# HanzhiC/TexPose

Measured on AMD Instinct MI355X. Metric: rendered rays/sec (480x640x128 samples) + train iters/sec, higher is better.
Workload: dtype f32 carried as 2xf16 (f16x3 products, f32 accumulate); 1 GPU; Duck-like synthetic scene 480x640, 128 samples/ray, batch=1 image per GPU, forward render (render_by_slices mode='val', all pixels), per-sample outputs materialised; samples_per_ray=128, mlp_precision=f16x3, parallelism=images sharded across 1 GPU(s), no collective

## Files before the change

### texpose_amd/csrc/gen_wide_asm.py

```python
#!/usr/bin/env python3
import sys

NCH = 115

VB = 160
def F_hi(slot): return VB + 8 * slot
def F_lo(slot): return VB + 8 * slot + 4
XB = [VB + 32, VB + 48]
T = VB + 64
VR = VB + 68
HACC = VB + 72
CLOBBER_V = list(range(XB[0], VR + 3))
BA, BB = 92, 94
CLOBBER_S = [BA, BA + 1, BB, BB + 1]
SET = {"P": 0, "Q": 128}


def vr(lo, n=4):
    return "v[%d:%d]" % (lo, lo + n - 1)


def ar(set_base, tile):
    lo = set_base + 16 * tile
    return "a[%d:%d]" % (lo, lo + 15)
# ... 100 lines not shown


def dma_base():
    return ["s_lshl_b32 %[t0], %[dch], 15",
            "s_add_u32 s%d, %%[stream_lo], %%[t0]" % BA,
            "s_addc_u32 s%d, %%[stream_hi], 0" % (BA + 1),
            "s_add_u32 s%d, s%d, 0x1000" % (BB, BA),
            "s_addc_u32 s%d, s%d, 0" % (BB + 1, BA + 1)]


def dma_piece(e, k, dma_slot):
    if k == 0:
        e("s_mov_b32 m0, %%[m%da]" % dma_slot)
        e("s_nop 0")
    elif k == 4:
        e("s_add_i32 m0, %%[m%da], 0x1000" % dma_slot)
        e("s_nop 0")
    base = "s[%d:%d]" % ((BA, BA + 1) if k < 4 else (BB, BB + 1))
    e("global_load_lds_dwordx4 %%[laneoff], %s offset:%d" % (base, (k & 3) * 1024))


def ring_epilogue(e, n_chunks):
    e("s_waitcnt lgkmcnt(0)")
    e("s_add_i32 %%[chunk], %%[chunk], %d" % n_chunks)
    e("s_cmp_ge_i32 %[chunk], %[nch]")
    e("s_cselect_b32 %[t0], %[nch], 0")
    e("s_sub_i32 %[chunk], %[chunk], %[t0]")
    e("s_add_i32 %%[buf], %%[buf], %d" % (n_chunks % 3))
    e("s_cmp_ge_i32 %[buf], 3")
    e("s_cselect_b32 %[t0], 3, 0")
    e("s_sub_i32 %[buf], %[buf], %[t0]")


def refill(e, slot, pair, npairs, cur, nxt):
    addr, off = (VR + cur, pair * 2048) if pair < npairs else (VR + nxt, (pair - npairs) * 2048)
    e("ds_read_b128 %s, v%d offset:%d" % (vr(F_hi(slot)), addr, off))
    e("ds_read_b128 %s, v%d offset:%d" % (vr(F_lo(slot)), addr, off + 1024))


def publish(e, young):
    e("s_waitcnt vmcnt(%d) lgkmcnt(0)" % young)
    e("s_barrier")


def chunk_groups(e, npairs, ts, mf, fill, free_after, pieces_per_group, tail=None, head=None, young_extra=0):
    ngroups = npairs // 2
    cur, nxt, dma = ts % 3, (ts + 1) % 3, (ts + 2) % 3
    pub_group = (npairs - 4) // 2
    for g in range(ngroups):
        q = 2 * g
        sa, sb = q % 4, (q + 1) % 4
        lines = mf(g)
        gaps = fill(g)
        e("s_waitcnt lgkmcnt(4)")
        for i in range(6):
            e(lines[i])
            if i == 0:
                for k in range(pieces_per_group):
                    dma_piece(e, g * pieces_per_group + k, dma)
                if head is not None:
                    for ins in head(g):
                        e(ins)
            if i < 5:
                for ins in gaps[i]:
                    e(ins)
            if i + 1 == free_after[0]:
                if g == pub_group:
                    publish(e, (g + 1) * pieces_per_group + young_extra)
                refill(e, sa, q + 4, npairs, cur, nxt)
            if i + 1 == free_after[1]:
                refill(e, sb, q + 5, npairs, cur, nxt)
        if tail is not None:
            for ins in tail(g):
                e(ins)


def advance_dch():
    return ["s_add_i32 %[dch], %[dch], 1", "s_cmp_eq_u32 %[dch], %[nch]", "s_cselect_b32 %[dch], 0, %[dch]"]


def gen_wide(src, dst, rec=None):
    L = []
    e = L.append
    ring_prologue(e)
    cvf = (lambda *a: conv_rec(*a, mask=(rec == "mask"))) if rec else conv
    if rec:
        e("s_mov_b64 s[%d:%d], %%[rbase]" % (RB, RB + 1))
    for g in range(8):
        for ins in cvf(src, 0, g, 0):
            e(ins)
    if rec:
        for ins in rec_reads(src, 0):
            e(ins)
    for ins in dma_base():
        e(ins)
    for ts in range(8):
        bank = ts & 1

        def mf(g, bank=bank):
            s, t = g >> 2, (2 * g) & 7
            sa, sb = (2 * g) % 4, (2 * g + 1) % 4
            xh, xl = vr(XB[bank] + s * 4), vr(XB[bank] + 8 + s * 4)
            d0, d1 = ar(dst, t), ar(dst, t + 1)
            return [mfma(d0, vr(F_hi(sa)), xh), mfma(d1, vr(F_hi(sb)), xh), mfma(d0, vr(F_hi(sa)), xl),
                    mfma(d1, vr(F_hi(sb)), xl), mfma(d0, vr(F_lo(sa)), xh), mfma(d1, vr(F_lo(sb)), xh)]

        def fill(g, ts=ts, bank=bank):
            if rec:
                first, mid1, mid2, mid3, last = [], [], [], [], []
                if 1 <= g <= 4:
                    first = [rec_store(src, ts, g - 1)]
                if g == 5:
                    first = rec_advance()
                if g == 7 and ts < 7:
                    rd = rec_reads(src, ts + 1)
                    mid2, mid3 = mid2 + rd[0:2], mid3 + rd[2:4]
                    if rec == "mask" and not (ts & 1):
                        last = last + rec_mask_store(ts >> 1)
                if ts == 7:
                    return [first, mid1, mid2, mid3, last]
                cv = conv_rec(src, ts + 1, g, bank ^ 1, mask=(rec == "mask"))
                if rec == "mask":
                    return [first + cv[0:4], mid1 + cv[4:9], cv[9:14] + mid2, cv[14:18] + mid3, cv[18:19] + last]
                return [first + cv[0:4], mid1 + cv[4:8], cv[8:12] + mid2, cv[12:15] + mid3, last]
            if ts == 7:
                return [[], [], [], [], []]
            cv = conv(src, ts + 1, g, bank ^ 1)
            return [[], cv[0:4], cv[4:8], cv[8:12], cv[12:13]]

        def tail(g, ts=ts):
            out = []
            if ts < 7:
                if 1 <= g <= 3:
                    out.append(advance_dch()[g - 1])
                if g == 7:
                    out += dma_base()
            return out

        def head(g, ts=ts):
            if g != (6 if rec else 0):
                return []
            return ["ds_read_b128 a[%d:%d], %%[nbias] offset:%d" % (src + 16 * ts + 4 * k, src + 16 * ts + 4 * k + 3, ts * 64 + k * 16)
                    for k in range(4)]

        extra = 0
        if rec:
            extra = 4 + (1 if (ts & 1) and rec == "mask" else 0)
        chunk_groups(e, 16, ts, mf, fill, (5, 6), 1, tail, head, young_extra=extra)
    ring_epilogue(e, 8)
    return L


def gen_extra(dst, ks):
    L = []
    e = L.append
    ring_prologue(e)
    for s in range(ks):
        e("ds_read_b128 %s, %%[stage] offset:%d" % (vr(XB[0] + s * 4), s * 8192))
        e("ds_read_b128 %s, %%[stage] offset:%d" % (vr(XB[0] + 8 + s * 4), s * 8192 + 4096))
    for ins in dma_base():
        e(ins)
    e("s_waitcnt lgkmcnt(0)")

    def mf(g):
        s, t = g >> 2, (2 * g) & 7
        sa, sb = (2 * g) % 4, (2 * g + 1) % 4
        xh, xl = vr(XB[0] + s * 4), vr(XB[0] + 8 + s * 4)
        d0, d1 = ar(dst, t), ar(dst, t + 1)
        return [mfma(d0, vr(F_hi(sa)), xh), mfma(d1, vr(F_hi(sb)), xh), mfma(d0, vr(F_hi(sa)), xl),
                mfma(d1, vr(F_hi(sb)), xl), mfma(d0, vr(F_lo(sa)), xh), mfma(d1, vr(F_lo(sb)), xh)]

    chunk_groups(e, 8 * ks, 0, mf, lambda g: [[], [], [], [], []], (5, 6), 2 // ks)
    ring_epilogue(e, 1)
    return L


def gen_head(src, rec=False):
    L = []
    e = L.append
    ring_prologue(e)
    if rec:
# ... 366 lines not shown

        tail = advance_dch() + dma_base() if c < 3 else []
        chunk16(e, lg, c, 4, dst, lambda s, b=b: vr(XB[b] + 4 * s), fill, tail)
    ring_epilogue(e, 4)
    return L


def gen_extra16(dst, ks):
    L = []
    e = L.append
    lg = Lgkm()
    ring_prologue(e)
    for s in range(ks):
        e("ds_read_b128 %s, %%[stage] offset:%d" % (vr(XB[0] + 4 * s), s * 8192))
    for ins in dma_base():
        e(ins)
    e("s_waitcnt lgkmcnt(0)")
    chunk16(e, lg, 0, ks, dst, lambda s: vr(XB[0] + 4 * s), lambda q: [])
    ring_epilogue(e, 1)
    return L


def emit_macro(out, name, comment, lines):
    out.append("// " + comment)
    out.append("#define %s \\" % name)
    out.append(" \\\n".join('    "%s\\n"' % l for l in lines))
    out.append("")


def main():
    out = ["// GENERATED by gen_wide_asm.py -- do not edit.  See that file for the schedule.", "#pragma once",
           "#define TP_ASM_CLOBBERS " + ", ".join(['"v%d"' % v for v in CLOBBER_V] + ['"s%d"' % r for r in CLOBBER_S] + ['"a%d"' % a for a in range(256)]),
           "#define TP_ASM_ALL_AGPRS " + ", ".join('"a%d"' % a for a in range(256)),
           '#define TP_ASM_REC_CLOBBERS "v%d", "s%d", "s%d", "vcc"' % (MK, RB, RB + 1)]
    for s, d in (("Q", "P"), ("P", "Q")):
        emit_macro(out, "TP_ASM_WIDE_%s%s" % (s, d), "256 -> 256 layer: set %s -> set %s" % (s, d), gen_wide(SET[s], SET[d]))
        emit_macro(out, "TP_ASM_WIDE_%s%s_REC" % (s, d), "256 -> 256 layer: set %s -> set %s, recording set %s (values + ReLU sign words)" % (s, d, s),
                   gen_wide(SET[s], SET[d], rec="mask"))
    emit_macro(out, "TP_ASM_WIDE_QP_RECNM", "256 -> 256 layer: set Q -> set P, recording set Q (values only: the trunk feature)",
               gen_wide(SET["Q"], SET["P"], rec="nomask"))
    for d in ("P", "Q"):
        for ks in (1, 2):
            emit_macro(out, "TP_ASM_EXTRA%d_%s" % (ks, d), "%d extra k-step(s) into set %s" % (ks, d), gen_extra(SET[d], ks))
        emit_macro(out, "TP_ASM_HEAD_%s" % d, "narrow head over relu(set %s)" % d, gen_head(SET[d]))
        emit_macro(out, "TP_ASM_HEAD_%s_REC" % d, "narrow head over relu(set %s), recording set %s" % (d, d), gen_head(SET[d], rec=True))
        emit_macro(out, "TP_ASM_INIT_%s" % d, "seed set %s with the bias block" % d, gen_init(SET[d]))
        for t in range(8):
            emit_macro(out, "TP_ASM_READ_%s%d" % (d, t), "tile %d of set %s -> v[232:247]" % (t, d), gen_read_tile(SET[d], t))
    emit_macro(out, "TP_ASM_HEADV_P1", "fp32 VALU head, 1 row, over relu(set P)", gen_head_valu(SET["P"], HEADTAB_SIGMA))
    emit_macro(out, "TP_ASM_HEADV_P5", "fp32 VALU head, 5 rows, over relu(set P)", gen_head_valu(SET["P"], HEADTAB_TRANS))
    emit_macro(out, "TP_ASM_HEADV_Q3", "fp32 VALU head, 3 rows, over relu(set Q)", gen_head_valu(SET["Q"], HEADTAB_RGB))
    out.append("#define TP_HEADTAB_OFFSETS {%s}" % ", ".join(str(v) for v in HEADTAB_SIGMA + HEADTAB_TRANS + HEADTAB_RGB))
    emit_macro(out, "TP_ASM_STASH_Q", "set Q -> v[32:159]", gen_stash(SET["Q"]))
    emit_macro(out, "TP_ASM_RESTORE_P", "v[32:159] -> set P", gen_restore(SET["P"]))
    for s, d in (("Q", "P"), ("P", "Q")):
        emit_macro(out, "TP_ASM_WIDE16_%s%s" % (s, d), "f16: 256 -> 256 layer: set %s -> set %s" % (s, d), gen_wide16(SET[s], SET[d]))
    for d in ("P", "Q"):
        for ks in (1, 4):
            emit_macro(out, "TP_ASM_EXTRA16_%d_%s" % (ks, d), "f16: %d extra k-step(s) into set %s" % (ks, d), gen_extra16(SET[d], ks))
    emit_macro(out, "TP_ASM_DG_NARROW_P", "data gradient: set P = W3^T d (one k-step)", gen_dg_narrow(SET["P"]))
    emit_macro(out, "TP_ASM_DG_WIDE_PQ", "data gradient: set Q = W^T gated(set P), recording gated(set P)", gen_dg_wide(SET["P"], SET["Q"]))
    emit_macro(out, "TP_ASM_DG_WIDE_QP", "data gradient: set P = W^T gated(set Q), recording gated(set Q)", gen_dg_wide(SET["Q"], SET["P"]))
    emit_macro(out, "TP_ASM_DG_FINISH_P", "data gradient: record gated(set P)", gen_dg_finish(SET["P"]))
    sys.stdout.write("\n".join(out) + "\n")


if __name__ == "__main__":
    main()
```

### texpose_amd/csrc/mlp_fwd_f16x3.hip

```cpp
#include "mlp_mma.h"
#include "wide_asm.inc.h"
#include <type_traits>

namespace {
using namespace tp_layout;
using namespace tp_mma;

using half8 = __attribute__((ext_vector_type(8))) _Float16;
using half2v = __attribute__((ext_vector_type(2))) __fp16;

constexpr int kBiasPad = (kBiasFloats + 63) / 64 * 64;
constexpr int kStageHalves = 5 * 2 * kThreads * 8;

constexpr int kBufs = 3;
constexpr int kSaveFloats = 8 * kThreads;
constexpr int kLdsBytes = kBufs * kChunkFloats * 4 + kBiasPad * 4 + kStageHalves * 2 + kSaveFloats * 4;
constexpr float kInvScale = 1.0f / (float)(1 << kF16WeightShift);

using u32x4 = __attribute__((ext_vector_type(4))) unsigned int;
__device__ __forceinline__ half8 pack8(const half2v (&p)[4]) {
  const u32x4 w = {__builtin_bit_cast(unsigned int, p[0]), __builtin_bit_cast(unsigned int, p[1]),
                   __builtin_bit_cast(unsigned int, p[2]), __builtin_bit_cast(unsigned int, p[3])};
  return __builtin_bit_cast(half8, w);
}
// ... 28 lines not shown
  for (int q = 0; q < kDepth; ++q) frag_fetch(f, q, l + q * kPairHalves);
}

struct Guard { half2v m = {(__fp16)0.0f, (__fp16)0.0f}; };

__device__ __forceinline__ float softplus(float x) { return x > 20.0f ? x : log1pf(expf(x)); }
__device__ __forceinline__ float sigmoid(float x) { return 1.0f / (1.0f + expf(-x)); }


struct AsmCtx { unsigned lane16, laneoff, ldswave, stream_lo, stream_hi, bias0, stage0; int nch; };
__device__ __forceinline__ AsmCtx asm_ctx_now(const float* packed, int nch = kNumChunks) {
  extern __shared__ __attribute__((aligned(16))) float lds_base[];
  int tid = threadIdx.x;
  asm volatile("" : "+v"(tid));
  const unsigned lane = (unsigned)tid & 63u, hh = ((unsigned)tid >> 5) & 1u;
  const unsigned wave = (unsigned)__builtin_amdgcn_readfirstlane(tid >> 6);
  AsmCtx c;
  const unsigned lds0 = (unsigned)(uintptr_t)AS3(lds_base);
  c.lane16 = lds0 + lane * 16u;
  c.laneoff = lane * 16u;
  c.ldswave = lds0 + wave * 8192u;
  const uint64_t sw = (uint64_t)(uintptr_t)(packed + wave * 2048);
  c.stream_lo = (unsigned)sw;
  c.stream_hi = (unsigned)(sw >> 32);
  const unsigned bias_lds = lds0 + (unsigned)(kBufs * kChunkFloats) * 4u;
  c.bias0 = bias_lds + hh * 512u;
  c.stage0 = bias_lds + (unsigned)kBiasPad * 4u + (unsigned)tid * 16u;
  c.nch = nch;
  return c;
}
#define TP_RING(f)                                                                                                     \
  "+{v[160:163]}"(f.h[0]), "+{v[164:167]}"(f.l[0]), "+{v[168:171]}"(f.h[1]), "+{v[172:175]}"(f.l[1]),                  \
      "+{v[176:179]}"(f.h[2]), "+{v[180:183]}"(f.l[2]), "+{v[184:187]}"(f.h[3]), "+{v[188:191]}"(f.l[3])
#define TP_RING_STATE                                                                                                  \
  [chunk] "+s"(chunk), [buf] "+s"(buf), [r0] "=&s"(r0), [r1] "=&s"(r1), [r2] "=&s"(r2), [m0a] "=&s"(m0a),              \
      [m1a] "=&s"(m1a), [m2a] "=&s"(m2a), [dch] "=&s"(dch), [t0] "=&s"(t0)
#define TP_RING_INPUTS(c)                                                                                              \
  [lane16] "v"(c.lane16), [laneoff] "v"(c.laneoff), [ldswave] "s"(__builtin_amdgcn_readfirstlane(c.ldswave)),         \
      [stream_lo] "s"(__builtin_amdgcn_readfirstlane(c.stream_lo)),                                                    \
      [stream_hi] "s"(__builtin_amdgcn_readfirstlane(c.stream_hi)), [nch] "s"(c.nch)
#define TP_ASM_HACC "v232", "v233", "v234", "v235", "v236", "v237", "v238", "v239", "v240", "v241", "v242", "v243", "v244", "v245", "v246", "v247"
#define TP_RING_LOCALS                                                                                                 \
  int chunk = __builtin_amdgcn_readfirstlane(p.chunk), buf = __builtin_amdgcn_readfirstlane(p.buf);                    \
  int r0, r1, r2, m0a, m1a, m2a, dch, t0
#define TP_RING_DONE                                                                                                   \
  p.chunk = chunk;                                                                                                     \
  p.buf = buf

#define TP_SF_OUT(F)                                                                                                   \
  "={v[32:47]}"(F[0]), "={v[48:63]}"(F[1]), "={v[64:79]}"(F[2]), "={v[80:95]}"(F[3]), "={v[96:111]}"(F[4]),            \
      "={v[112:127]}"(F[5]), "={v[128:143]}"(F[6]), "={v[144:159]}"(F[7])
#define TP_SF_IN(F)                                                                                                    \
  "{v[32:47]}"(F[0]), "{v[48:63]}"(F[1]), "{v[64:79]}"(F[2]), "{v[80:95]}"(F[3]), "{v[96:111]}"(F[4]),                 \
      "{v[112:127]}"(F[5]), "{v[128:143]}"(F[6]), "{v[144:159]}"(F[7])
__device__ __forceinline__ void asm_stash_q(f32x16 (&F)[8]) { asm volatile(TP_ASM_STASH_Q : TP_SF_OUT(F) : : TP_ASM_ALL_AGPRS); }
__device__ __forceinline__ void asm_restore_p(const f32x16 (&F)[8]) { asm volatile(TP_ASM_RESTORE_P : : TP_SF_IN(F) : TP_ASM_ALL_AGPRS); }
template <bool SRC_Q>
__device__ __forceinline__ void asm_wide(Pipe& p, Frag& f, Guard& amax, const AsmCtx& c, int next_li) {
  TP_RING_LOCALS;
  const float kinv = kInvScale;
  const unsigned mask = 0xFFFFE000u;
  const unsigned nbias = c.bias0 + (unsigned)next_li * 1024u;
  if constexpr (SRC_Q)
    asm volatile(TP_ASM_WIDE_QP : TP_RING(f), TP_RING_STATE, [amax] "+v"(amax.m)
                 : TP_RING_INPUTS(c), [kinv] "s"(kinv), [mask] "s"(mask), [nbias] "v"(nbias)
                 : TP_ASM_CLOBBERS, TP_ASM_HACC, "memory", "scc");
  else
    asm volatile(TP_ASM_WIDE_PQ : TP_RING(f), TP_RING_STATE, [amax] "+v"(amax.m)
                 : TP_RING_INPUTS(c), [kinv] "s"(kinv), [mask] "s"(mask), [nbias] "v"(nbias)
                 : TP_ASM_CLOBBERS, TP_ASM_HACC, "memory", "scc");
  TP_RING_DONE;
}

template <bool SRC_Q>
__device__ __forceinline__ void asm_wide16(Pipe& p, Frag& f, Guard& amax, const AsmCtx& c, int next_li) {
  TP_RING_LOCALS;
  const unsigned nbias = c.bias0 + (unsigned)next_li * 1024u;
  if constexpr (SRC_Q)
    asm volatile(TP_ASM_WIDE16_QP : TP_RING(f), TP_RING_STATE, [amax] "+v"(amax.m)
                 : TP_RING_INPUTS(c), [nbias] "v"(nbias) : TP_ASM_CLOBBERS, "memory", "scc");
  else
    asm volatile(TP_ASM_WIDE16_PQ : TP_RING(f), TP_RING_STATE, [amax] "+v"(amax.m)
                 : TP_RING_INPUTS(c), [nbias] "v"(nbias) : TP_ASM_CLOBBERS, "memory", "scc");
  TP_RING_DONE;
}

struct RecCtx { unsigned recw, recr, ro0, ro1, mkoff; const float* rbase; };
__device__ __forceinline__ RecCtx rec_ctx_now(float* saved, int64_t tile, int slot) {
  extern __shared__ __attribute__((aligned(16))) float lds_base[];
  int tid = threadIdx.x;
  asm volatile("" : "+v"(tid));
  const unsigned lane = (unsigned)tid & 63u, j = (unsigned)tid & 31u, hh = ((unsigned)tid >> 5) & 1u;
  const unsigned wave = (unsigned)__builtin_amdgcn_readfirstlane(tid >> 6);
  const unsigned stg = (unsigned)(uintptr_t)AS3(lds_base) + (unsigned)(kBufs * kChunkFloats + kBiasPad) * 4u + wave * 1024u;
  RecCtx c;
  c.recw = stg + ((4u * hh) * 32u + j) * 4u;
  c.recr = stg + lane * 16u;
  c.ro0 = (unsigned)blk_off(0 + (int)(lane >> 3), (int)(lane & 7u) * 4) * 4u;
  c.ro1 = (unsigned)blk_off(8 + (int)(lane >> 3), (int)(lane & 7u) * 4) * 4u;
  static_assert(blk_off(16 + 3, 12) == blk_off(3, 12) + 512 && blk_off(24 + 6, 20) == blk_off(8 + 6, 20) + 512,
                "units 2 / 3 of a record tile sit 16 rows behind units 0 / 1 with the same swizzle");
  c.mkoff = (unsigned)((kMaskOff + ((slot > 0 ? slot : 1) - 1) * 256 - slot * kBlockFloats) * 4) + lane * 4u;
  const float* base = saved + (tile * 4 + (int64_t)wave) * (int64_t)kSavedGroupFloats + (int64_t)slot * kBlockFloats;
  const uint64_t b = (uint64_t)(uintptr_t)base;
  c.rbase = reinterpret_cast<const float*>((uint64_t)(unsigned)__builtin_amdgcn_readfirstlane((int)(unsigned)b) |
                                           ((uint64_t)(unsigned)__builtin_amdgcn_readfirstlane((int)(unsigned)(b >> 32)) << 32));
  return c;
}
#define TP_REC_INPUTS(r)                                                                                               \
  [recw] "v"(r.recw), [recr] "v"(r.recr), [ro0] "v"(r.ro0), [ro1] "v"(r.ro1), [mkoff] "v"(r.mkoff), [rbase] "s"(r.rbase)

template <class L>
constexpr int rec_kind_of() {
  if constexpr (std::is_same_v<L, int>) return 0;
  else return L::value == T0 ? 2 : (L::value == T1 || L::value == T2 || L::value == R1 || L::value == R2) ? 1 : 0;
}

template <bool SRC_Q, bool MASK>
__device__ __forceinline__ void asm_wide_rec(Pipe& p, Frag& f, Guard& amax, const AsmCtx& c, int next_li, const RecCtx& r) {
  TP_RING_LOCALS;
  const float kinv = kInvScale;
  const unsigned mask = 0xFFFFE000u;
  const unsigned nbias = c.bias0 + (unsigned)next_li * 1024u;
  static_assert(SRC_Q || MASK, "the mask-free variant exists for set Q only");
#define TP_WIDE_REC(TXT)                                                                                               \
  asm volatile(TXT : TP_RING(f), TP_RING_STATE, [amax] "+v"(amax.m)                                                    \
               : TP_RING_INPUTS(c), [kinv] "s"(kinv), [mask] "s"(mask), [nbias] "v"(nbias), TP_REC_INPUTS(r)           \
               : TP_ASM_CLOBBERS, TP_ASM_REC_CLOBBERS, "memory", "scc")
  if constexpr (SRC_Q && MASK) TP_WIDE_REC(TP_ASM_WIDE_QP_REC);
  else if constexpr (SRC_Q) TP_WIDE_REC(TP_ASM_WIDE_QP_RECNM);
  else TP_WIDE_REC(TP_ASM_WIDE_PQ_REC);
#undef TP_WIDE_REC
  TP_RING_DONE;
}

template <int KS, bool DST_P>
__device__ __forceinline__ void asm_extra(Pipe& p, Frag& f, const AsmCtx& c, int ks0) {
  TP_RING_LOCALS;
  const unsigned stage = c.stage0 + (unsigned)ks0 * 8192u;
#define TP_EXTRA(TXT)                                                                                                  \
  asm volatile(TXT : TP_RING(f), TP_RING_STATE : TP_RING_INPUTS(c), [stage] "v"(stage)                  \
               : TP_ASM_CLOBBERS, "memory", "scc")
  if constexpr (KS == 1 && DST_P) TP_EXTRA(TP_ASM_EXTRA1_P);
  else if constexpr (KS == 2 && DST_P) TP_EXTRA(TP_ASM_EXTRA2_P);
  else if constexpr (KS == 1) TP_EXTRA(TP_ASM_EXTRA1_Q);
  else TP_EXTRA(TP_ASM_EXTRA2_Q);
#undef TP_EXTRA
  TP_RING_DONE;
}

template <int KS, bool DST_P>
__device__ __forceinline__ void asm_extra16(Pipe& p, Frag& f, const AsmCtx& c, int ks0) {
  TP_RING_LOCALS;
  const unsigned stage = c.stage0 + (unsigned)ks0 * 8192u;
#define TP_EXTRA16(TXT)                                                                                                \
  asm volatile(TXT : TP_RING(f), TP_RING_STATE : TP_RING_INPUTS(c), [stage] "v"(stage) : TP_ASM_CLOBBERS, "memory", "scc")
  if constexpr (KS == 1 && DST_P) TP_EXTRA16(TP_ASM_EXTRA16_1_P);
  else if constexpr (KS == 4 && DST_P) TP_EXTRA16(TP_ASM_EXTRA16_4_P);
  else if constexpr (KS == 1) TP_EXTRA16(TP_ASM_EXTRA16_1_Q);
  else TP_EXTRA16(TP_ASM_EXTRA16_4_Q);
#undef TP_EXTRA16
  TP_RING_DONE;
}

template <bool SRC_P>
__device__ __forceinline__ f32x16 asm_head(Pipe& p, Frag& f, Guard& amax, const AsmCtx& c, float kinv = kInvScale) {
  TP_RING_LOCALS;
  const unsigned mask = 0xFFFFE000u;
  f32x16 acc;
  if constexpr (SRC_P)
    asm volatile(TP_ASM_HEAD_P : TP_RING(f), TP_RING_STATE, [amax] "+v"(amax.m), "=&{v[232:247]}"(acc)
                 : TP_RING_INPUTS(c), [kinv] "s"(kinv), [mask] "s"(mask) : TP_ASM_CLOBBERS, "memory", "scc");
  else
    asm volatile(TP_ASM_HEAD_Q : TP_RING(f), TP_RING_STATE, [amax] "+v"(amax.m), "=&{v[232:247]}"(acc)
                 : TP_RING_INPUTS(c), [kinv] "s"(kinv), [mask] "s"(mask) : TP_ASM_CLOBBERS, "memory", "scc");
  TP_RING_DONE;
  return acc;
}

struct Head4 { float a0, a1, a2, a3; };
template <bool SRC_P>
__device__ __forceinline__ Head4 asm_head_rec(Pipe& p, Frag& f, Guard& amax, const AsmCtx& c, const RecCtx& r) {
  TP_RING_LOCALS;
  const float kinv = kInvScale;
  const unsigned mask = 0xFFFFE000u;
  Head4 h;
#define TP_HEAD_REC(TXT)                                                                                               \
  asm volatile(TXT : TP_RING(f), TP_RING_STATE, [amax] "+v"(amax.m), "=&{v232}"(h.a0), "=&{v233}"(h.a1),               \
                     "=&{v234}"(h.a2), "=&{v235}"(h.a3)                                                                \
               : TP_RING_INPUTS(c), [kinv] "s"(kinv), [mask] "s"(mask), TP_REC_INPUTS(r)                               \
               : TP_ASM_CLOBBERS, TP_ASM_REC_CLOBBERS, "v236", "v237", "v238", "v239", "v240", "v241", "v242", "v243", \
                 "v244", "v245", "v246", "v247", "memory", "scc")
  if constexpr (SRC_P) TP_HEAD_REC(TP_ASM_HEAD_P_REC);
  else TP_HEAD_REC(TP_ASM_HEAD_Q_REC);
#undef TP_HEAD_REC
  TP_RING_DONE;
  return h;
}

struct Head5 { float r0, r1, r2, r3, r4; };
template <int WHICH>
__device__ __forceinline__ Head5 asm_head_valu(const Pipe& p, Frag& f, const AsmCtx& c) {
  int tid = threadIdx.x;
  asm volatile("" : "+v"(tid));
  const unsigned hw = c.stage0 - (unsigned)tid * 16u + (((unsigned)tid >> 5) & 1u) * 16u;
  const int buf = __builtin_amdgcn_readfirstlane(p.buf);
  int t0;
  Head5 h;
#define TP_HEADV(TXT)                                                                                                  \
  asm volatile(TXT : TP_RING(f), [t0] "=&s"(t0), "=&{v232}"(h.r0), "=&{v233}"(h.r1), "=&{v234}"(h.r2), "=&{v235}"(h.r3), \
                     "=&{v236}"(h.r4)                                                                                  \
               : [hw] "v"(hw), [lane16] "v"(c.lane16), [buf] "s"(buf)                                                  \
               : TP_ASM_CLOBBERS, "v231", "v237", "v238", "v239", "v240", "v241", "v242", "v243", "v244", "v245", "v246", "v247", \
                 "memory", "scc")
  if constexpr (WHICH == 0) TP_HEADV(TP_ASM_HEADV_P1);
  else if constexpr (WHICH == 1) TP_HEADV(TP_ASM_HEADV_P5);
  else TP_HEADV(TP_ASM_HEADV_Q3);
#undef TP_HEADV
  return h;
}

template <bool DST_P>
__device__ __forceinline__ void asm_init(const AsmCtx& c, int li) {
  const unsigned bias = c.bias0 + (unsigned)li * 1024u;
  if constexpr (DST_P) asm volatile(TP_ASM_INIT_P :: [bias] "v"(bias) : TP_ASM_CLOBBERS, "memory");
  else asm volatile(TP_ASM_INIT_Q :: [bias] "v"(bias) : TP_ASM_CLOBBERS, "memory");
}

struct Params {
  const float* packed;
  const float* center; const float* ray; const float* depth;
  const float* points; const float* ray_unit;
  const float* lat_trans; const float* lat_light;
  int B, R, N;
  int64_t n_samples, n_tiles;
  float* rgb; float* density; float* uncert; float* saved; float* workspace; int* status;
  const float* density_noise;
  unsigned int* act_max;
  const float* ray_bias;
};

__device__ __forceinline__ void stage(_Float16* st, int tid, int ks, int j, float v) {
  const _Float16 hi = (_Float16)v;
  st[((ks * 2 + 0) * kThreads + tid) * 8 + j] = hi;
  st[((ks * 2 + 1) * kThreads + tid) * 8 + j] = (_Float16)(v - (float)hi);
}

__device__ __forceinline__ void stage_slot(_Float16* st, int tid_lo, int slot, float v) {
  const int ks = slot >> 4, owner = tid_lo | ((slot & 8) << 2), jj = slot & 7;
  const _Float16 hi = (_Float16)v;
  st[((ks * 2 + 0) * kThreads + owner) * 8 + jj] = hi;
  st[((ks * 2 + 1) * kThreads + owner) * 8 + jj] = (_Float16)(v - (float)hi);
}

#define TP_THREAD_IDS                                                                                                  \
  int tid = threadIdx.x;                                                                                               \
  asm volatile("" : "+v"(tid));                                                                                        \
  const int lane = tid & 63, j = tid & 31, hh = (tid >> 5) & 1;                                                        \
  const int wave = __builtin_amdgcn_readfirstlane(tid >> 6);                                                           \
// ... 2 lines not shown

template <bool SAVE, bool RB = false, bool F16 = false>
__global__ __launch_bounds__(kThreads, 1) void mlp_fwd_f16x3_kernel(Params P) {
  static_assert(!(SAVE && RB), "the ray-bias stream has no recording variant");
  static_assert(!(SAVE && F16), "the single-product arithmetic is inference only");
  constexpr int NCH = F16 ? (RB ? kNumChunks16RB : kNumChunks16) : (RB ? kNumChunksRB : kNumChunks);
  constexpr int BIAS_NCH = RB ? kNumChunksRB : kNumChunks;
  constexpr float kSetScale = F16 ? 1.0f : (float)(1 << kF16WeightShift);
#define TP_CTX asm_ctx_now(P.packed, NCH)
  extern __shared__ __attribute__((aligned(16))) float lds[];
  const int tid = threadIdx.x, lane = tid & 63, wave = tid >> 6;
  float* bias_lds = lds + kBufs * kChunkFloats;
  _Float16* st = reinterpret_cast<_Float16*>(bias_lds + kBiasPad);

  Pipe p;
  p.stream = P.packed; p.lds = lds; p.chunk = 0; p.buf = 0; p.wave = __builtin_amdgcn_readfirstlane(wave); p.lane = lane;
  for (int i = tid; i < kBiasFloats; i += kThreads)
    bias_lds[i] = P.packed[(size_t)BIAS_NCH * kChunkFloats + i] * (i < kHeadBiasOff ? kSetScale : 1.0f);
  if constexpr (RB) {
    constexpr int kHeadTabOff[kRbHeadRows] = TP_HEADTAB_OFFSETS;
    const float* tab = P.packed + kRbAuxOff + kRbAuxHeads;
    for (int i = tid; i < kRbHeadRows * 256; i += kThreads)
      *reinterpret_cast<float*>(reinterpret_cast<char*>(st) + kHeadTabOff[i >> 8] + (i & 255) * 4) =
          tab[i] * ((float)(1 << kF16WeightShift) / kSetScale);
  }
  dma_chunk(p, 0, 0);
  dma_chunk(p, 1, 1);
  __syncthreads();
  Frag frag;
  frag_prime(p, frag);
#ifdef TP_TRACE
  const long long tr_start = tick();
#endif
  asm_init<true>(TP_CTX, L0);

  for (int64_t tile = blockIdx.x; tile < P.n_tiles; tile += gridDim.x) {
    TR_BEGIN(pro);
    TP_THREAD_IDS;
    const int64_t s_raw = tile * 128 + wave * 32 + j;
    const bool live = s_raw < P.n_samples;
    const int64_t s = live ? s_raw : 0;
    const int64_t q = s / P.N;
    const int b = (int)(q / P.R);
    {
      float x0, x1, x2, vu0, vu1, vu2;
      if (P.center != nullptr) {
        const float z = P.depth[s];
        const float d0 = P.ray[3 * q + 0], d1 = P.ray[3 * q + 1], d2 = P.ray[3 * q + 2];
        x0 = tp::add_rn(P.center[3 * q + 0], tp::mul_rn(d0, z));
        x1 = tp::add_rn(P.center[3 * q + 1], tp::mul_rn(d1, z));
        x2 = tp::add_rn(P.center[3 * q + 2], tp::mul_rn(d2, z));
        float nrm = tp::add_rn(0.f, tp::mul_rn(d0, d0));
        nrm = tp::add_rn(nrm, tp::mul_rn(d1, d1));
        nrm = tp::add_rn(nrm, tp::mul_rn(d2, d2));
        const float den = fmaxf(sqrtf(nrm), 1e-12f);
        vu0 = tp::div_rn(d0, den); vu1 = tp::div_rn(d1, den); vu2 = tp::div_rn(d2, den);
      } else {
        x0 = P.points[3 * s + 0]; x1 = P.points[3 * s + 1]; x2 = P.points[3 * s + 2];
        vu0 = P.ray_unit[3 * s + 0]; vu1 = P.ray_unit[3 * s + 1]; vu2 = P.ray_unit[3 * s + 2];
      }
      save[0 * kThreads] = x0; save[1 * kThreads] = x1; save[2 * kThreads] = x2;
      if constexpr (!RB) {
        save[3 * kThreads] = vu0; save[4 * kThreads] = vu1; save[5 * kThreads] = vu2;
        save[6 * kThreads] = __int_as_float(b);
      } else {
        const int64_t qt = (tile * 128) / P.N;
        bias_lds[R0 * 256 + tid] = P.ray_bias[(size_t)P.B * 512 + (size_t)qt * 256 + tid] * (kSetScale * kInvScale);
        bias_lds[T0 * 256 + tid] = P.ray_bias[(size_t)(qt / P.R) * 512 + tid] * (kSetScale * kInvScale);
      }
    }
    asm_init<false>(TP_CTX, L1);
    TR_END(4, pro);
    f32x16 SF[8];
    Guard amax;
    float sig_s, rgb_s[3], ta0, ta1, ta2, ta3;
    const float* hbias = bias_lds + kHeadBiasOff;

    const auto head = [&](auto which_tag, auto after) {
      constexpr int which = decltype(which_tag)::value;
      TR_BEGIN(h);
      float a0, a1, a2, a3;
      if constexpr (SAVE && which != 0) {
        Head4 h4;
        if constexpr (which == 2) h4 = asm_head_rec<false>(p, frag, amax, TP_CTX, rec_ctx_now(P.saved, tile, SV_R2));
        else h4 = asm_head_rec<true>(p, frag, amax, TP_CTX, rec_ctx_now(P.saved, tile, SV_T2));
        a0 = h4.a0; a1 = h4.a1; a2 = h4.a2; a3 = h4.a3;
        TR_END(7, h);
      } else if constexpr (RB) {
        const Head5 h5 = asm_head_valu<which>(p, frag, TP_CTX);
        TR_END(7, h);
        TP_THREAD_IDS;
        a0 = (which == 1 && hh) ? h5.r4 : h5.r0; a1 = h5.r1; a2 = h5.r2; a3 = h5.r3;
      } else {
        f32x16 a;
        if constexpr (which == 2) a = asm_head<false>(p, frag, amax, TP_CTX, 1.0f / kSetScale);
        else a = asm_head<true>(p, frag, amax, TP_CTX, 1.0f / kSetScale);
        TR_END(7, h);
        a0 = a[0]; a1 = a[1]; a2 = a[2]; a3 = a[3];
      }
      after();
      if (which == 0) {
        float dn = 0.0f;
        if (P.density_noise != nullptr) {
          TP_THREAD_IDS;
          int64_t sn = tile * 128 + wave * 32 + j;
          if (sn >= P.n_samples) sn = P.n_samples - 1;
          dn = P.density_noise[sn];
        }
        sig_s = softplus(fmaf(a0, kInvScale, hbias[0]) + dn);
      } else if (which == 1) {
        ta0 = a0; ta1 = a1; ta2 = a2; ta3 = a3;
      } else {
        rgb_s[0] = sigmoid(fmaf(a0, kInvScale, hbias[6])); rgb_s[1] = sigmoid(fmaf(a1, kInvScale, hbias[7]));
        rgb_s[2] = sigmoid(fmaf(a2, kInvScale, hbias[8]));
      }
    };

    const auto layer = [&](auto even_tag, auto li_arg) {
      constexpr bool EVEN = decltype(even_tag)::value;
      const int li = li_arg;
      constexpr int REC = SAVE ? rec_kind_of<decltype(li_arg)>() : 0;
      if (!EVEN && li == L7) head(std::integral_constant<int, 0>{}, [] {});
      if (!EVEN && li == R0)
        head(std::integral_constant<int, 1>{}, [&] {
          TR_BEGIN(rl);
          asm_restore_p(SF);
          TR_END(10, rl);
        });

      if (li != L0) {
        TR_BEGIN(w);
        const int next_li = li + 1 == kNumWide ? 0 : li + 1;
        if constexpr (REC == 2) asm_wide_rec<true, false>(p, frag, amax, TP_CTX, next_li, rec_ctx_now(P.saved, tile, SV_FEAT));
        else if constexpr (REC == 1) asm_wide_rec<EVEN, true>(p, frag, amax, TP_CTX, next_li, rec_ctx_now(P.saved, tile, li - 1 - L7));
        else if constexpr (F16) asm_wide16<EVEN>(p, frag, amax, TP_CTX, next_li);
        else asm_wide<EVEN>(p, frag, amax, TP_CTX, next_li);
        TR_END(3, w);
      }

      if (EVEN && (li == L0 || li == L4)) {
        TR_BEGIN(pe);
        if (li == L0) {
          TP_THREAD_IDS;
          const float x0 = save[0 * kThreads], x1 = save[1 * kThreads], x2 = save[2 * kThreads];
          const int ca = 2 * hh;
          tp::SinCos64 ea = tp::sincos_f64(tp::mul_rn(hh ? x2 : x0, 3.14159274101257324f));
          tp::SinCos64 eb = tp::sincos_f64(tp::mul_rn(x1, 3.14159274101257324f));
#pragma unroll
          for (int l = 0; l < 10; ++l) {
            stage_slot(st, tid & ~32, 20 * ca + l, (float)ea.s);
            stage_slot(st, tid & ~32, 20 * ca + 10 + l, (float)ea.c);
            stage_slot(st, tid & ~32, 20 + 10 * hh + l, (float)(hh ? eb.c : eb.s));
            if (l < 9) { tp::sincos_double(ea); tp::sincos_double(eb); }
          }
          if (hh) {
            stage(st, tid, 3, 4, x0); stage(st, tid, 3, 5, x1); stage(st, tid, 3, 6, x2); stage(st, tid, 3, 7, 0.0f);
          }
        }
        TR_END(5, pe);
        TR_BEGIN(w);
        if constexpr (F16) {
          asm_extra16<4, true>(p, frag, TP_CTX, 0);
        } else {
          asm_extra<2, true>(p, frag, TP_CTX, 0);
          asm_extra<2, true>(p, frag, TP_CTX, 2);
        }
        TR_END(3, w);
      } else if (RB && EVEN && li == T0) {
      } else if (RB && !EVEN && li == R0) {
        TR_BEGIN(r0s);
        TP_THREAD_IDS;
        if (hh == 0) {
          save[0 * kThreads] = sigmoid(fmaf(ta0, kInvScale, hbias[1]));
          save[1 * kThreads] = sigmoid(fmaf(ta1, kInvScale, hbias[2]));
          save[2 * kThreads] = sigmoid(fmaf(ta2, kInvScale, hbias[3]));
          save[3 * kThreads] = softplus(fmaf(ta3, kInvScale, hbias[4]));
        } else {
          save[0 * kThreads] = softplus(fmaf(ta0, kInvScale, hbias[5]));
        }
        TR_END(6, r0s);
        TR_BEGIN(w);
        if constexpr (F16) asm_extra16<1, false>(p, frag, TP_CTX, 3);
        else asm_extra<1, false>(p, frag, TP_CTX, 3);
        TR_END(3, w);
      } else if (EVEN && li == T0) {
        TR_BEGIN(t0s);
        TP_THREAD_IDS;
        const int bt = __float_as_int(save[6 * kThreads]);
#pragma unroll
        for (int jj = 0; jj < 8; ++jj) stage(st, tid, 0, jj, P.lat_trans[bt * 16 + 8 * hh + jj]);
        TR_END(13, t0s);
        TR_BEGIN(w);
        if constexpr (F16) asm_extra16<1, true>(p, frag, TP_CTX, 0);
        else asm_extra<1, true>(p, frag, TP_CTX, 0);
        TR_END(3, w);
      } else if (!EVEN && li == R0) {
        TR_BEGIN(r0s);
        TP_THREAD_IDS;
        float* sx = SAVE ? P.saved + (tile * 4 + wave) * (int64_t)kSavedGroupFloats + SV_EX * kBlockFloats : nullptr;
        const float x0 = save[0 * kThreads], x1 = save[1 * kThreads], x2 = save[2 * kThreads];
        const float vu0 = save[3 * kThreads], vu1 = save[4 * kThreads], vu2 = save[5 * kThreads];
        const int br = __float_as_int(save[6 * kThreads]);
        {
          const int ca = 2 * hh;
          tp::SinCos64 ea = tp::sincos_f64(tp::mul_rn(hh ? vu2 : vu0, 3.14159274101257324f));
          tp::SinCos64 eb = tp::sincos_f64(tp::mul_rn(vu1, 3.14159274101257324f));
#pragma unroll
          for (int l = 0; l < 4; ++l) {
            const float sa = (float)ea.s, cav = (float)ea.c, vb = (float)(hh ? eb.c : eb.s);
            const int s0 = 3 + 8 * ca + l, s1 = 3 + 8 + 4 * hh + l;
            stage_slot(st, tid & ~32, s0, sa);
            stage_slot(st, tid & ~32, s0 + 4, cav);
            stage_slot(st, tid & ~32, s1, vb);
            if (SAVE && live) { sx[blk_off(s0, j)] = sa; sx[blk_off(s0 + 4, j)] = cav; sx[blk_off(s1, j)] = vb; }
            if (l < 3) { tp::sincos_double(ea); tp::sincos_double(eb); }
          }
        }
        if (hh == 0) {
          stage(st, tid, 0, 0, vu0); stage(st, tid, 0, 1, vu1); stage(st, tid, 0, 2, vu2);
          if (SAVE && live) { sx[blk_off(0, j)] = vu0; sx[blk_off(1, j)] = vu1; sx[blk_off(2, j)] = vu2; }
        } else {
          stage(st, tid, 1, 3, x0); stage(st, tid, 1, 4, x1); stage(st, tid, 1, 5, x2);
          stage(st, tid, 1, 6, P.lat_light[br * 48 + 0]); stage(st, tid, 1, 7, P.lat_light[br * 48 + 1]);
          if (SAVE && live) { sx[blk_off(27, j)] = x0; sx[blk_off(28, j)] = x1; sx[blk_off(29, j)] = x2; }
        }
#pragma unroll
        for (int ks = 2; ks < 5; ++ks) {
          float lv[8];
#pragma unroll
          for (int jj = 0; jj < 8; ++jj) {
            const int slot = 16 * ks + 8 * hh + jj;
            lv[jj] = slot < 78 ? P.lat_light[br * 48 + slot - 30] : 0.0f;
          }
          half8 hi8, lo8;
#pragma unroll
          for (int jj = 0; jj < 8; ++jj) {
            hi8[jj] = (_Float16)lv[jj];
            lo8[jj] = (_Float16)(lv[jj] - (float)hi8[jj]);
          }
          *reinterpret_cast<half8*>(st + ((ks * 2 + 0) * kThreads + tid) * 8) = hi8;
          *reinterpret_cast<half8*>(st + ((ks * 2 + 1) * kThreads + tid) * 8) = lo8;
        }
        if (hh == 0) {
          save[0 * kThreads] = sigmoid(fmaf(ta0, kInvScale, hbias[1]));
          save[1 * kThreads] = sigmoid(fmaf(ta1, kInvScale, hbias[2]));
          save[2 * kThreads] = sigmoid(fmaf(ta2, kInvScale, hbias[3]));
          save[3 * kThreads] = softplus(fmaf(ta3, kInvScale, hbias[4]));
        } else {
          save[0 * kThreads] = softplus(fmaf(ta0, kInvScale, hbias[5]));
        }
        TR_END(6, r0s);
        TR_BEGIN(w);
        if constexpr (F16) {
          asm_extra16<4, false>(p, frag, TP_CTX, 0);
          asm_extra16<1, false>(p, frag, TP_CTX, 4);
        } else {
          asm_extra<2, false>(p, frag, TP_CTX, 0);
          asm_extra<2, false>(p, frag, TP_CTX, 2);
          asm_extra<1, false>(p, frag, TP_CTX, 4);
        }
        TR_END(3, w);
      }

      if (!EVEN && li == L7) {
        TR_BEGIN(vc);
        asm_stash_q(SF);
        TR_END(9, vc);
      }
    };

    if constexpr (SAVE) {
#pragma nounroll
      for (int pr = 0; pr < 4; ++pr) {
        layer(std::true_type{}, 2 * pr);
        layer(std::false_type{}, 2 * pr + 1);
      }
      layer(std::true_type{}, std::integral_constant<int, T0>{});
      layer(std::false_type{}, std::integral_constant<int, T1>{});
      layer(std::true_type{}, std::integral_constant<int, T2>{});
      layer(std::false_type{}, std::integral_constant<int, R0>{});
      layer(std::true_type{}, std::integral_constant<int, R1>{});
      layer(std::false_type{}, std::integral_constant<int, R2>{});
    } else {
#pragma nounroll
      for (int pr = 0; pr < kNumWide / 2; ++pr) {
        layer(std::true_type{}, 2 * pr);
        layer(std::false_type{}, 2 * pr + 1);
      }
    }
    head(std::integral_constant<int, 2>{}, [] {});

    TR_BEGIN(o);
// ... 361 lines not shown
```

Before: 2.122 million rays/s.

## Carry tile-0 activations across wide layers in bank-0 registers

Adds carry variants of the 256->256 wide-layer asm. The last k-step processes output tiles in tile-major order so the next layer's first input tile (conversion, ReLU, amax) can be produced in the MMA gaps and kept in the XB0 VGPRs. A following carry-enabled layer then skips its own serial conversion prologue, hiding that VALU work behind MFMAs. In exchange the XB0 registers must stay live across the extra and head asm blocks, which adds register pressure and makes the schedule more intricate.

```diff
diff --git a/texpose_amd/csrc/gen_wide_asm.py b/texpose_amd/csrc/gen_wide_asm.py
--- a/texpose_amd/csrc/gen_wide_asm.py
+++ b/texpose_amd/csrc/gen_wide_asm.py
@@ -156,8 +156,15 @@
     e("s_sub_i32 %[buf], %[buf], %[t0]")
 
 
-def refill(e, slot, pair, npairs, cur, nxt):
-    addr, off = (VR + cur, pair * 2048) if pair < npairs else (VR + nxt, (pair - npairs) * 2048)
+def tile_major(q):
+    return 8 * ((q >> 1) & 1) + 2 * (q >> 2) + (q & 1)
+
+
+def refill(e, slot, pair, npairs, cur, nxt, order=None, next_order=None):
+    if pair < npairs:
+        addr, off = VR + cur, (order(pair) if order else pair) * 2048
+    else:
+        addr, off = VR + nxt, (next_order(pair - npairs) if next_order else pair - npairs) * 2048
     e("ds_read_b128 %s, v%d offset:%d" % (vr(F_hi(slot)), addr, off))
     e("ds_read_b128 %s, v%d offset:%d" % (vr(F_lo(slot)), addr, off + 1024))
 
@@ -167,7 +174,8 @@
     e("s_barrier")
 
 
-def chunk_groups(e, npairs, ts, mf, fill, free_after, pieces_per_group, tail=None, head=None, young_extra=0):
+def chunk_groups(e, npairs, ts, mf, fill, free_after, pieces_per_group, tail=None, head=None, young_extra=0, order=None,
+                 next_order=None):
     ngroups = npairs // 2
     cur, nxt, dma = ts % 3, (ts + 1) % 3, (ts + 2) % 3
     pub_group = (npairs - 4) // 2
@@ -191,9 +199,9 @@
             if i + 1 == free_after[0]:
                 if g == pub_group:
                     publish(e, (g + 1) * pieces_per_group + young_extra)
-                refill(e, sa, q + 4, npairs, cur, nxt)
+                refill(e, sa, q + 4, npairs, cur, nxt, order, next_order)
             if i + 1 == free_after[1]:
-                refill(e, sb, q + 5, npairs, cur, nxt)
+                refill(e, sb, q + 5, npairs, cur, nxt, order, next_order)
         if tail is not None:
             for ins in tail(g):
                 e(ins)
@@ -203,16 +211,45 @@
     return ["s_add_i32 %[dch], %[dch], 1", "s_cmp_eq_u32 %[dch], %[nch]", "s_cselect_b32 %[dch], 0, %[dch]"]
 
 
-def gen_wide(src, dst, rec=None):
+GT = HACC
+
+CARRY_QUOTA = [2, 4, 4, 4, 1]
+
+
+def carry_tail(dst):
+    cv = []
+    for k in range(8):
+        c = conv(dst, 0, k, 0)
+        xh = XB[0] + (k >> 2) * 4 + (k & 3)
+        cv += c[:-1] + ["v_pk_max_f16 v%d, v%d, v%d" % (GT, GT, xh)]
+    cv += ["v_and_b32 v%d, %%[post], v%d" % (GT, GT), "v_pk_max_f16 %%[amax], %%[amax], v%d" % GT]
+    out, pos = {}, 0
+    for g in range(2, 8):
+        for i, n in enumerate(CARRY_QUOTA):
+            out[(g, i)] = cv[pos:pos + n]
+            pos += n
+    assert pos == len(cv)
+    out[(1, 4)] = ["v_mov_b32 v%d, 0" % GT]
+    return out
+
+
+def gen_wide(src, dst, rec=None, carry=False):
+    assert not (rec and carry)
     L = []
     e = L.append
     ring_prologue(e)
     cvf = (lambda *a: conv_rec(*a, mask=(rec == "mask"))) if rec else conv
     if rec:
         e("s_mov_b64 s[%d:%d], %%[rbase]" % (RB, RB + 1))
+    if carry:
+        e("s_cmp_lg_u32 %[pre], 0")
+        e("s_cbranch_scc1 .Lwide_pre_%=")
     for g in range(8):
         for ins in cvf(src, 0, g, 0):
             e(ins)
+    if carry:
+        e(".Lwide_pre_%=:")
+        ctail = carry_tail(dst)
     if rec:
         for ins in rec_reads(src, 0):
             e(ins)
@@ -221,15 +258,19 @@
     for ts in range(8):
         bank = ts & 1
 
-        def mf(g, bank=bank):
-            s, t = g >> 2, (2 * g) & 7
+        tm = carry and ts == 7
+
+        def mf(g, bank=bank, tm=tm):
+            s, t = (g & 1, 2 * (g >> 1)) if tm else (g >> 2, (2 * g) & 7)
             sa, sb = (2 * g) % 4, (2 * g + 1) % 4
             xh, xl = vr(XB[bank] + s * 4), vr(XB[bank] + 8 + s * 4)
             d0, d1 = ar(dst, t), ar(dst, t + 1)
             return [mfma(d0, vr(F_hi(sa)), xh), mfma(d1, vr(F_hi(sb)), xh), mfma(d0, vr(F_hi(sa)), xl),
                     mfma(d1, vr(F_hi(sb)), xl), mfma(d0, vr(F_lo(sa)), xh), mfma(d1, vr(F_lo(sb)), xh)]
 
-        def fill(g, ts=ts, bank=bank):
+        def fill(g, ts=ts, bank=bank, tm=tm):
+            if tm:
+                return [ctail.get((g, i), []) for i in range(5)]
             if rec:
                 first, mid1, mid2, mid3, last = [], [], [], [], []
                 if 1 <= g <= 4:
@@ -270,7 +311,8 @@
         extra = 0
         if rec:
             extra = 4 + (1 if (ts & 1) and rec == "mask" else 0)
-        chunk_groups(e, 16, ts, mf, fill, (5, 6), 1, tail, head, young_extra=extra)
+        chunk_groups(e, 16, ts, mf, fill, (5, 6), 1, tail, head, young_extra=extra, order=tile_major if tm else None,
+                     next_order=tile_major if carry and ts == 6 else None)
     ring_epilogue(e, 8)
     return L
 
@@ -703,9 +745,12 @@
     out = ["// GENERATED by gen_wide_asm.py -- do not edit.  See that file for the schedule.", "#pragma once",
            "#define TP_ASM_CLOBBERS " + ", ".join(['"v%d"' % v for v in CLOBBER_V] + ['"s%d"' % r for r in CLOBBER_S] + ['"a%d"' % a for a in range(256)]),
            "#define TP_ASM_ALL_AGPRS " + ", ".join('"a%d"' % a for a in range(256)),
-           '#define TP_ASM_REC_CLOBBERS "v%d", "s%d", "s%d", "vcc"' % (MK, RB, RB + 1)]
+           '#define TP_ASM_REC_CLOBBERS "v%d", "s%d", "s%d", "vcc"' % (MK, RB, RB + 1),
+           "#define TP_ASM_CLOBBERS_XB0 " + ", ".join(['"v%d"' % v for v in CLOBBER_V if not XB[0] <= v < XB[1]] + ['"s%d"' % r for r in CLOBBER_S] + ['"a%d"' % a for a in range(256)])]
     for s, d in (("Q", "P"), ("P", "Q")):
         emit_macro(out, "TP_ASM_WIDE_%s%s" % (s, d), "256 -> 256 layer: set %s -> set %s" % (s, d), gen_wide(SET[s], SET[d]))
+        emit_macro(out, "TP_ASM_WIDE_%s%s_CARRY" % (s, d), "256 -> 256 layer: set %s -> set %s, tile-0 operands carried in / out in bank 0" % (s, d),
+                   gen_wide(SET[s], SET[d], carry=True))
         emit_macro(out, "TP_ASM_WIDE_%s%s_REC" % (s, d), "256 -> 256 layer: set %s -> set %s, recording set %s (values + ReLU sign words)" % (s, d, s),
                    gen_wide(SET[s], SET[d], rec="mask"))
     emit_macro(out, "TP_ASM_WIDE_QP_RECNM", "256 -> 256 layer: set Q -> set P, recording set Q (values only: the trunk feature)",
diff --git a/texpose_amd/csrc/mlp_fwd_f16x3.hip b/texpose_amd/csrc/mlp_fwd_f16x3.hip
--- a/texpose_amd/csrc/mlp_fwd_f16x3.hip
+++ b/texpose_amd/csrc/mlp_fwd_f16x3.hip
@@ -84,7 +84,16 @@
 #define TP_RING(f)                                                                                                     \
   "+{v[160:163]}"(f.h[0]), "+{v[164:167]}"(f.l[0]), "+{v[168:171]}"(f.h[1]), "+{v[172:175]}"(f.l[1]),                  \
       "+{v[176:179]}"(f.h[2]), "+{v[180:183]}"(f.l[2]), "+{v[184:187]}"(f.h[3]), "+{v[188:191]}"(f.l[3])
-#define TP_RING_STATE                                                                                                  \
+struct XB0 { u32x4 r[4]; };
+struct NoXB0 {};
+#define TP_XB0(x) "+{v[192:195]}"(x.r[0]), "+{v[196:199]}"(x.r[1]), "+{v[200:203]}"(x.r[2]), "+{v[204:207]}"(x.r[3])
+#define TP_XB0_OPT(x) , TP_XB0(x)
+__device__ __forceinline__ void xb0_undef(XB0& x) {
+  asm volatile("" : "={v[192:195]}"(x.r[0]), "={v[196:199]}"(x.r[1]), "={v[200:203]}"(x.r[2]), "={v[204:207]}"(x.r[3]));
+}
+__device__ __forceinline__ void xb0_undef(NoXB0&) {}
+constexpr unsigned kCarryLayers = (1u << L1) | (1u << L2) | (1u << L3) | (1u << L5) | (1u << L7) | (1u << T0) | (1u << T1) | (1u << R1);
+#define TP_RING_STATE                                                                                               \
   [chunk] "+s"(chunk), [buf] "+s"(buf), [r0] "=&s"(r0), [r1] "=&s"(r1), [r2] "=&s"(r2), [m0a] "=&s"(m0a),              \
       [m1a] "=&s"(m1a), [m2a] "=&s"(m2a), [dch] "=&s"(dch), [t0] "=&s"(t0)
 #define TP_RING_INPUTS(c)                                                                                              \
@@ -123,6 +132,23 @@
                  : TP_ASM_CLOBBERS, TP_ASM_HACC, "memory", "scc");
   TP_RING_DONE;
 }
+template <bool SRC_Q>
+__device__ __forceinline__ void asm_wide(Pipe& p, Frag& f, Guard& amax, const AsmCtx& c, int next_li, XB0& xb, bool pre_set, bool post_set) {
+  TP_RING_LOCALS;
+  const float kinv = kInvScale;
+  const unsigned mask = 0xFFFFE000u;
+  const unsigned nbias = c.bias0 + (unsigned)next_li * 1024u;
+  const int pre = pre_set ? 1 : 0, post = post_set ? -1 : 0;
+  if constexpr (SRC_Q)
+    asm volatile(TP_ASM_WIDE_QP_CARRY : TP_RING(f), TP_RING_STATE, [amax] "+v"(amax.m), TP_XB0(xb)
+                 : TP_RING_INPUTS(c), [kinv] "s"(kinv), [mask] "s"(mask), [nbias] "v"(nbias), [pre] "s"(pre), [post] "s"(post)
+                 : TP_ASM_CLOBBERS_XB0, TP_ASM_HACC, "memory", "scc");
+  else
+    asm volatile(TP_ASM_WIDE_PQ_CARRY : TP_RING(f), TP_RING_STATE, [amax] "+v"(amax.m), TP_XB0(xb)
+                 : TP_RING_INPUTS(c), [kinv] "s"(kinv), [mask] "s"(mask), [nbias] "v"(nbias), [pre] "s"(pre), [post] "s"(post)
+                 : TP_ASM_CLOBBERS_XB0, TP_ASM_HACC, "memory", "scc");
+  TP_RING_DONE;
+}
 
 template <bool SRC_Q>
 __device__ __forceinline__ void asm_wide16(Pipe& p, Frag& f, Guard& amax, const AsmCtx& c, int next_li) {
@@ -186,18 +212,23 @@
   TP_RING_DONE;
 }
 
-template <int KS, bool DST_P>
-__device__ __forceinline__ void asm_extra(Pipe& p, Frag& f, const AsmCtx& c, int ks0) {
+template <int KS, bool DST_P, class XB>
+__device__ __forceinline__ void asm_extra(Pipe& p, Frag& f, const AsmCtx& c, int ks0, XB& xb) {
   TP_RING_LOCALS;
   const unsigned stage = c.stage0 + (unsigned)ks0 * 8192u;
+#define TP_EXTRA_(TXT, XBOPT, CLOB)                                                                                    \
+  asm volatile(TXT : TP_RING(f), TP_RING_STATE XBOPT : TP_RING_INPUTS(c), [stage] "v"(stage) : CLOB, "memory", "scc")
 #define TP_EXTRA(TXT)                                                                                                  \
-  asm volatile(TXT : TP_RING(f), TP_RING_STATE : TP_RING_INPUTS(c), [stage] "v"(stage)                  \
-               : TP_ASM_CLOBBERS, "memory", "scc")
+  do {                                                                                                                 \
+    if constexpr (std::is_same_v<XB, XB0>) TP_EXTRA_(TXT, TP_XB0_OPT(xb), TP_ASM_CLOBBERS_XB0);                        \
+    else TP_EXTRA_(TXT, , TP_ASM_CLOBBERS);                                                                            \
+  } while (0)
   if constexpr (KS == 1 && DST_P) TP_EXTRA(TP_ASM_EXTRA1_P);
   else if constexpr (KS == 2 && DST_P) TP_EXTRA(TP_ASM_EXTRA2_P);
   else if constexpr (KS == 1) TP_EXTRA(TP_ASM_EXTRA1_Q);
   else TP_EXTRA(TP_ASM_EXTRA2_Q);
 #undef TP_EXTRA
+#undef TP_EXTRA_
   TP_RING_DONE;
 }
 
@@ -251,32 +282,43 @@
 }
 
 struct Head5 { float r0, r1, r2, r3, r4; };
-template <int WHICH>
-__device__ __forceinline__ Head5 asm_head_valu(const Pipe& p, Frag& f, const AsmCtx& c) {
+template <int WHICH, class XB>
+__device__ __forceinline__ Head5 asm_head_valu(const Pipe& p, Frag& f, const AsmCtx& c, XB& xb) {
   int tid = threadIdx.x;
   asm volatile("" : "+v"(tid));
   const unsigned hw = c.stage0 - (unsigned)tid * 16u + (((unsigned)tid >> 5) & 1u) * 16u;
   const int buf = __builtin_amdgcn_readfirstlane(p.buf);
   int t0;
   Head5 h;
+#define TP_HEADV_(TXT, XBOPT, CLOB)                                                                                    \
+  asm volatile(TXT : TP_RING(f), [t0] "=&s"(t0), "=&{v232}"(h.r0), "=&{v233}"(h.r1), "=&{v234}"(h.r2), "=&{v235}"(h.r3), \
+                     "=&{v236}"(h.r4) XBOPT                                                                            \
+               : [hw] "v"(hw), [lane16] "v"(c.lane16), [buf] "s"(buf)                                                  \
+               : CLOB, "v231", "v237", "v238", "v239", "v240", "v241", "v242", "v243", "v244", "v245", "v246", "v247", \
+                 "memory", "scc")
 #define TP_HEADV(TXT)                                                                                                  \
-  asm volatile(TXT : TP_RING(f), [t0] "=&s"(t0), "=&{v232}"(h.r0), "=&{v233}"(h.r1), "=&{v234}"(h.r2), "=&{v235}"(h.r3), \
-                     "=&{v236}"(h.r4)                                                                                  \
-               : [hw] "v"(hw), [lane16] "v"(c.lane16), [buf] "s"(buf)                                                  \
-               : TP_ASM_CLOBBERS, "v231", "v237", "v238", "v239", "v240", "v241", "v242", "v243", "v244", "v245", "v246", "v247", \
-                 "memory", "scc")
+  do {                                                                                                                 \
+    if constexpr (std::is_same_v<XB, XB0>) TP_HEADV_(TXT, TP_XB0_OPT(xb), TP_ASM_CLOBBERS_XB0);                        \
+    else TP_HEADV_(TXT, , TP_ASM_CLOBBERS);                                                                            \
+  } while (0)
   if constexpr (WHICH == 0) TP_HEADV(TP_ASM_HEADV_P1);
   else if constexpr (WHICH == 1) TP_HEADV(TP_ASM_HEADV_P5);
   else TP_HEADV(TP_ASM_HEADV_Q3);
 #undef TP_HEADV
+#undef TP_HEADV_
   return h;
 }
 
-template <bool DST_P>
+template <bool DST_P, class XB = NoXB0>
 __device__ __forceinline__ void asm_init(const AsmCtx& c, int li) {
   const unsigned bias = c.bias0 + (unsigned)li * 1024u;
-  if constexpr (DST_P) asm volatile(TP_ASM_INIT_P :: [bias] "v"(bias) : TP_ASM_CLOBBERS, "memory");
-  else asm volatile(TP_ASM_INIT_Q :: [bias] "v"(bias) : TP_ASM_CLOBBERS, "memory");
+  if constexpr (std::is_same_v<XB, XB0>) {
+    if constexpr (DST_P) asm volatile(TP_ASM_INIT_P :: [bias] "v"(bias) : TP_ASM_CLOBBERS_XB0, "memory");
+    else asm volatile(TP_ASM_INIT_Q :: [bias] "v"(bias) : TP_ASM_CLOBBERS_XB0, "memory");
+  } else {
+    if constexpr (DST_P) asm volatile(TP_ASM_INIT_P :: [bias] "v"(bias) : TP_ASM_CLOBBERS, "memory");
+    else asm volatile(TP_ASM_INIT_Q :: [bias] "v"(bias) : TP_ASM_CLOBBERS, "memory");
+  }
 }
 
 struct Params {
@@ -345,7 +387,10 @@
 #ifdef TP_TRACE
   const long long tr_start = tick();
 #endif
-  asm_init<true>(TP_CTX, L0);
+  using XB = std::conditional_t<RB && !F16, XB0, NoXB0>;
+  XB xb;
+  xb0_undef(xb);
+  asm_init<true, XB>(TP_CTX, L0);
 
   for (int64_t tile = blockIdx.x; tile < P.n_tiles; tile += gridDim.x) {
     TR_BEGIN(pro);
@@ -382,7 +427,7 @@
         bias_lds[T0 * 256 + tid] = P.ray_bias[(size_t)(qt / P.R) * 512 + tid] * (kSetScale * kInvScale);
       }
     }
-    asm_init<false>(TP_CTX, L1);
+    asm_init<false, XB>(TP_CTX, L1);
     TR_END(4, pro);
     f32x16 SF[8];
     Guard amax;
@@ -400,7 +445,8 @@
         a0 = h4.a0; a1 = h4.a1; a2 = h4.a2; a3 = h4.a3;
         TR_END(7, h);
       } else if constexpr (RB) {
-        const Head5 h5 = asm_head_valu<which>(p, frag, TP_CTX);
+        const Head5 h5 = asm_head_valu<which>(p, frag, TP_CTX, xb);
+        xb0_undef(xb);
         TR_END(7, h);
         TP_THREAD_IDS;
         a0 = (which == 1 && hh) ? h5.r4 : h5.r0; a1 = h5.r1; a2 = h5.r2; a3 = h5.r3;
@@ -447,7 +493,8 @@
         if constexpr (REC == 2) asm_wide_rec<true, false>(p, frag, amax, TP_CTX, next_li, rec_ctx_now(P.saved, tile, SV_FEAT));
         else if constexpr (REC == 1) asm_wide_rec<EVEN, true>(p, frag, amax, TP_CTX, next_li, rec_ctx_now(P.saved, tile, li - 1 - L7));
         else if constexpr (F16) asm_wide16<EVEN>(p, frag, amax, TP_CTX, next_li);
-        else asm_wide<EVEN>(p, frag, amax, TP_CTX, next_li);
+        else if constexpr (!RB) asm_wide<EVEN>(p, frag, amax, TP_CTX, next_li);
+        else asm_wide<EVEN>(p, frag, amax, TP_CTX, next_li, xb, (kCarryLayers >> (li - 1)) & 1u, (kCarryLayers >> li) & 1u);
         TR_END(3, w);
       }
 
@@ -475,8 +522,8 @@
         if constexpr (F16) {
           asm_extra16<4, true>(p, frag, TP_CTX, 0);
         } else {
-          asm_extra<2, true>(p, frag, TP_CTX, 0);
-          asm_extra<2, true>(p, frag, TP_CTX, 2);
+          asm_extra<2, true>(p, frag, TP_CTX, 0, xb);
+          asm_extra<2, true>(p, frag, TP_CTX, 2, xb);
         }
         TR_END(3, w);
       } else if (RB && EVEN && li == T0) {
@@ -494,7 +541,7 @@
         TR_END(6, r0s);
         TR_BEGIN(w);
         if constexpr (F16) asm_extra16<1, false>(p, frag, TP_CTX, 3);
-        else asm_extra<1, false>(p, frag, TP_CTX, 3);
+        else asm_extra<1, false>(p, frag, TP_CTX, 3, xb);
         TR_END(3, w);
       } else if (EVEN && li == T0) {
         TR_BEGIN(t0s);
@@ -505,7 +552,7 @@
         TR_END(13, t0s);
         TR_BEGIN(w);
         if constexpr (F16) asm_extra16<1, true>(p, frag, TP_CTX, 0);
-        else asm_extra<1, true>(p, frag, TP_CTX, 0);
+        else asm_extra<1, true>(p, frag, TP_CTX, 0, xb);
         TR_END(3, w);
       } else if (!EVEN && li == R0) {
         TR_BEGIN(r0s);
@@ -568,9 +615,9 @@
           asm_extra16<4, false>(p, frag, TP_CTX, 0);
           asm_extra16<1, false>(p, frag, TP_CTX, 4);
         } else {
-          asm_extra<2, false>(p, frag, TP_CTX, 0);
-          asm_extra<2, false>(p, frag, TP_CTX, 2);
-          asm_extra<1, false>(p, frag, TP_CTX, 4);
+          asm_extra<2, false>(p, frag, TP_CTX, 0, xb);
+          asm_extra<2, false>(p, frag, TP_CTX, 2, xb);
+          asm_extra<1, false>(p, frag, TP_CTX, 4, xb);
         }
         TR_END(3, w);
       }
```

Result: no change. 2.122 million rays/s (-0.0%).
